# ChumpChief/FluidFramework

Hardware: AMD Instinct MI355X
Metric: sequenced ops applied/sec (whole node) + achieved HBM GB/s, conflict-farm replay (higher is better)
Workload: dtype int32

## Files before the change

### fluidframework_amd/csrc/kernels.h

```cpp
#pragma once

#include <hip/hip_runtime.h>

#include "../../include/fmt.h"

namespace fmt_mt {
struct AdjustTables;
struct LocalTables;
}

namespace fmt_kernels {

size_t mapLwwLdsBytes(uint32_t keyBound);
bool mapLwwNeedsScratch(uint32_t keyBound);
size_t mapSparseLdsBytes();
hipError_t launchMapSparse(const fmt_map_op* ops, const uint64_t* offsets, uint32_t nDocs, uint32_t keyBound,
                           fmt_map_entry* out, uint32_t* counts, int* error, int numCUs, hipStream_t stream);
hipError_t launchMapSparsePack(const fmt_map_entry* in, const uint64_t* offsets, const uint32_t* counts,
                               const uint64_t* packedOff, uint32_t nDocs, fmt_map_entry* packed, hipStream_t stream);
size_t mapPendingScratchBytes(uint64_t nEvents);
hipError_t launchMapPending(const fmt_map_local_op* events, const uint64_t* evOffs, const fmt_map_entry* seqEntries,
                            const uint64_t* seqOffs, const uint32_t* seqCounts, uint32_t nDocs, void* scratch,
                            const uint64_t* outBase, fmt_map_entry* out, uint32_t* outCounts, int32_t* outStatus,
                            hipStream_t stream);
// ... 5 lines not shown
  const uint64_t* docOpOffsets;
  uint32_t nDocs;
  const uint16_t* text;
  const uint32_t* docInit;
  const uint32_t* propsOff;
  const uint32_t* propsKv;
  uint32_t nPropsOps;
  const uint64_t* catchupOffsets;
  const fmt_mt_snapshot_doc* snapshots;
  const fmt_mt_snapshot_seg* snapshotSegs;
  const uint64_t* rmOrderOffsets;
  const fmt_mt_snapshot_info* snapshotInfo;
  const fmt_mt_stamp* snapshotStamps;
  uint64_t nSnapshotInfo;
  const fmt_mt_relpos* relpos;
  uint32_t nRelpos;
  uint32_t markerKey;
  const fmt_mt::AdjustTables* adj;
  const fmt_mt::LocalTables* loc = nullptr;
};

struct MtDeviceOut {
  fmt_mt_doc_result* headers;
  fmt_mt_leaf* leaves;
  uint16_t* chars;
  fmt_mt_propset* props;
  fmt_mt_catchup_range* catchup;
  fmt_mt_remove_order* rmOrder;
  uint32_t* ckpt;
  const fmt_mt_leaf* smallLeaves;
  const uint16_t* smallChars;
  uint16_t* legacyProps;
  uint32_t* hugeCkpt = nullptr;
};
size_t mergeTreeCheckpointBytes();

struct SumView {
  const fmt_mt_leaf* leaves;
  const uint16_t* chars;
  const fmt_mt_propset* props;
  const uint16_t* legacyProps;
  const uint32_t* cls;
  const uint64_t* rmHi;
};
struct SumRun {
  uint32_t len;
  uint16_t props;
  uint16_t flags;
};
struct SumDocOut {
  unsigned long long run_off, text_off;
  uint32_t n_runs, n_units, status, pad;
};
hipError_t launchSummaryRuns(const fmt_mt_doc_result* hdrs, const SumView* views, uint32_t nDocs, SumRun* runs,
                             uint16_t* text, unsigned long long* cursors, SumDocOut* docOut, int numCUs,
                             hipStream_t stream);
struct GatherSpan {
  const uint32_t* src;
  uint64_t dstWord;
  uint32_t words, pad;
};
hipError_t launchGatherSpans(const GatherSpan* spans, uint32_t n, uint32_t* dst, int numCUs, hipStream_t stream);
hipError_t launchStateDigest(const fmt_mt_doc_result* hdrs, const SumView* views, uint32_t nDocs, uint64_t* out,
                             int numCUs, hipStream_t stream);

struct MtCaps {
  uint32_t leaves, chars, props;
};
MtCaps mergeTreeCaps(bool large);

hipError_t launchMergeTree(const MtDeviceBatch& batch, const MtDeviceOut& out, const uint32_t* docList,
                           uint32_t count, uint32_t* esc, uint32_t* esc2, uint32_t* esc3, uint32_t* esc4, int numCUs,
                           hipStream_t stream, bool obliterate, bool removeOrder, uint32_t* sched, bool adjust);

hipError_t launchMergeTreeLarge(const MtDeviceBatch& batch, const MtDeviceOut& out, const uint32_t* docList,
                                uint32_t count, int numCUs, hipStream_t stream, bool obliterate, bool removeOrder,
                                uint32_t* next, bool adjust, bool local = false);

hipError_t launchMergeTreeLocal(const MtDeviceBatch& batch, const MtDeviceOut& out, const uint32_t* docList,
                                uint32_t count, uint32_t* esc, uint32_t* esc2, int numCUs, hipStream_t stream,
                                uint32_t* sched, bool adjust = false);

int mergeTreeProfile(uint64_t* out, int n, bool reset);

}

namespace fmt_huge {
struct HugeState;
struct HugeInputs;
}

namespace fmt_kernels {

struct HugeOut {
  fmt_mt_doc_result* header;
  fmt_mt_leaf* leaves;
  uint64_t capLeaves;
  uint16_t* chars;
  uint64_t capChars;
  fmt_mt_propset* props;
  uint16_t* legacy;
  const uint32_t* cls;
  unsigned long long* prof;
  uint64_t* leavesHi;
};
size_t hugeLdsBytes();
// ... 5 lines not shown
```

### fluidframework_amd/csrc/mergetree.hip

```cpp
#define FMT_MT_COLLECT_DEFINE 1
#include "mergetree_kernel.h"

namespace fmt_kernels {

constexpr int kMtWaves = 4;

int mergeTreeProfileCompact(uint64_t* out, int n, bool reset);
int mergeTreeProfileMicro(uint64_t* out, int n, bool reset);
int mergeTreeProfileLarge(uint64_t* out, int n, bool reset);

int mergeTreeProfile(uint64_t* out, int n, bool reset) {
  for (int c = 0; c < n; c++) out[c] = 0;
  if (addTuProfile(out, n, reset) < 0 || mergeTreeProfileCompact(out, n, reset) < 0 ||
      mergeTreeProfileMicro(out, n, reset) < 0 || mergeTreeProfileLarge(out, n, reset) < 0)
    return -1;
  return fmt_mt::kPfCount;
}

MtCaps mergeTreeCaps(bool large) {
  if (large)
    return MtCaps{static_cast<uint32_t>(Slab<fmt_mt::LargeTier>::kLeaves), static_cast<uint32_t>(Slab<fmt_mt::LargeTier>::kChars),
                  static_cast<uint32_t>(Slab<fmt_mt::LargeTier>::kProps)};
  return MtCaps{static_cast<uint32_t>(Slab<fmt_mt::SmallTier>::kLeaves), static_cast<uint32_t>(Slab<fmt_mt::SmallTier>::kChars),
                static_cast<uint32_t>(Slab<fmt_mt::SmallTier>::kProps)};
}

size_t mergeTreeCheckpointBytes() { return sizeof(uint32_t) * fmt_mt::Doc<false, fmt_mt::CompactTier>::kCkptWords; }

hipError_t launchMergeTreeCompact(const MtDeviceBatch& batch, const MtDeviceOut& out, const uint32_t* docList,
                                  uint32_t count, uint32_t* esc, int numCUs, hipStream_t stream, uint32_t* next,
                                  bool obliterate, const uint32_t* countDev);
hipError_t launchMergeTreeMicro(const MtDeviceBatch& batch, const MtDeviceOut& out, const uint32_t* docList,
                                uint32_t count, uint32_t* esc, int numCUs, hipStream_t stream, uint32_t* next);

constexpr int kOrderBuckets = 64;
__global__ __launch_bounds__(1024) void orderByRemainingKernel(const uint32_t* __restrict__ in, uint32_t* __restrict__ out,
                                                               const fmt_mt_doc_result* __restrict__ headers,
                                                               const uint64_t* __restrict__ offs,
                                                               const uint32_t* __restrict__ ckpt, uint32_t ckptWords) {
  __shared__ uint32_t cnt[kOrderBuckets], base[kOrderBuckets], maxRem;
  const uint32_t n = in[0];
  if (threadIdx.x < kOrderBuckets) cnt[threadIdx.x] = 0;
  if (threadIdx.x == 0) maxRem = 0;
  __syncthreads();
  auto remaining = [&](uint32_t d) -> uint32_t {
    uint64_t first = offs[d];
    if (headers[d].status == fmt_mt::kCkptEscalate) {
      const uint32_t* h = ckpt + static_cast<size_t>(d) * ckptWords;
      first = h[0] | (static_cast<uint64_t>(h[1]) << 32);
    }
    const uint64_t r = offs[d + 1] - first;
    return r > 0xffffffffull ? 0xffffffffu : static_cast<uint32_t>(r);
  };
  for (uint32_t i = threadIdx.x; i < n; i += blockDim.x) atomicMax(&maxRem, remaining(in[1 + i]));
  __syncthreads();
  const uint64_t span = static_cast<uint64_t>(maxRem) + 1;
  auto bucket = [&](uint32_t r) -> uint32_t {
    return kOrderBuckets - 1 - static_cast<uint32_t>(static_cast<uint64_t>(r) * kOrderBuckets / span);
  };
  for (uint32_t i = threadIdx.x; i < n; i += blockDim.x) atomicAdd(&cnt[bucket(remaining(in[1 + i]))], 1u);
  __syncthreads();
  if (threadIdx.x == 0) {
    uint32_t s = 0;
    for (int b = 0; b < kOrderBuckets; b++) {
      base[b] = s;
      s += cnt[b];
    }
    out[0] = n;
  }
  __syncthreads();
  for (uint32_t i = threadIdx.x; i < n; i += blockDim.x) {
    const uint32_t d = in[1 + i];
    out[1 + atomicAdd(&base[bucket(remaining(d))], 1u)] = d;
  }
}

hipError_t launchMergeTree(const MtDeviceBatch& batch, const MtDeviceOut& out, const uint32_t* docList,
                           uint32_t count, uint32_t* esc, uint32_t* esc2, uint32_t* esc3, uint32_t* esc4, int numCUs,
                           hipStream_t stream, bool obliterate, bool removeOrder, uint32_t* sched, bool adjust) {
  using S = fmt_mt::SmallTier;
  uint32_t* n1 = sched ? sched + 1 : nullptr;
  if (adjust) {
    if (removeOrder)
      return launchTier<true, S, true, kMtWaves, 1, true>(batch, out, docList, count, esc, numCUs, stream, nullptr, n1);
    return launchTier<true, S, false, kMtWaves, 1, true>(batch, out, docList, count, esc, numCUs, stream, nullptr, n1);
  }
  if (obliterate && removeOrder)
    return launchTier<true, S, true, kMtWaves, 2>(batch, out, docList, count, esc, numCUs, stream, nullptr, n1);
  if (obliterate && (esc == nullptr || esc2 == nullptr))
    return launchTier<true, S, false, kMtWaves, 2>(batch, out, docList, count, esc, numCUs, stream, nullptr, n1);
  if (removeOrder)
    return launchTier<false, S, true, kMtWaves, 2>(batch, out, docList, count, esc, numCUs, stream, nullptr, n1);
  if (esc == nullptr || esc2 == nullptr)
    return launchTier<false, S, false, kMtWaves, 2>(batch, out, docList, count, esc, numCUs, stream, nullptr, n1);
  constexpr uint32_t kCkptWords = static_cast<uint32_t>(fmt_mt::Doc<false, fmt_mt::CompactTier>::kCkptWords);
  const bool order = esc3 != nullptr && out.ckpt != nullptr;
  hipError_t e;
  if (!obliterate && esc4 != nullptr) {
    e = launchMergeTreeMicro(batch, out, docList, count, esc2, numCUs, stream, sched ? sched + 3 : nullptr);
    if (e != hipSuccess) return e;
    uint32_t* list = esc2;
    if (order) {
      hipLaunchKernelGGL(orderByRemainingKernel, dim3(1), dim3(1024), 0, stream, esc2, esc3, out.headers,
                         batch.docOpOffsets, out.ckpt, kCkptWords);
      list = esc3;
    }
    e = launchMergeTreeCompact(batch, out, list + 1, count, esc4, numCUs, stream, sched, false, list);
    if (e != hipSuccess) return e;
    if (order) {
      hipLaunchKernelGGL(orderByRemainingKernel, dim3(1), dim3(1024), 0, stream, esc4, esc2, out.headers,
                         batch.docOpOffsets, out.ckpt, kCkptWords);
      list = esc2;
    } else {
      list = esc4;
    }
    return launchTier<false, S, false, kMtWaves, 2>(batch, out, list + 1, count, esc, numCUs, stream, list, n1);
  }
  e = launchMergeTreeCompact(batch, out, docList, count, esc2, numCUs, stream, sched, obliterate, nullptr);
  if (e != hipSuccess) return e;
  if (order) {
    hipLaunchKernelGGL(orderByRemainingKernel, dim3(1), dim3(1024), 0, stream, esc2, esc3, out.headers,
                       batch.docOpOffsets, out.ckpt, kCkptWords);
    esc2 = esc3;
  }
  if (obliterate)
    return launchTier<true, S, false, kMtWaves, 2>(batch, out, esc2 + 1, count, esc, numCUs, stream, esc2, n1);
  return launchTier<false, S, false, kMtWaves, 2>(batch, out, esc2 + 1, count, esc, numCUs, stream, esc2, n1);
}

}
```

### fluidframework_amd/csrc/mergetree_kernel.h

```cpp
#pragma once
#include <hip/hip_runtime.h>

#include "kernels.h"
#include "mt_engine.h"

namespace fmt_kernels {

static __device__ unsigned long long g_mtProfile[fmt_mt::kPfCount];

static inline int addTuProfile(uint64_t* out, int n, bool reset) {
  unsigned long long h[fmt_mt::kPfCount];
  if (hipMemcpyFromSymbol(h, HIP_SYMBOL(g_mtProfile), sizeof h) != hipSuccess) return -1;
  for (int c = 0; c < n && c < fmt_mt::kPfCount; c++) out[c] += h[c];
  if (reset) {
    unsigned long long z[fmt_mt::kPfCount] = {};
    if (hipMemcpyToSymbol(HIP_SYMBOL(g_mtProfile), z, sizeof z) != hipSuccess) return -1;
  }
  return fmt_mt::kPfCount;
}

template <class C>
struct Slab {
  static constexpr size_t kLeaves = C::kHbmChars ? 64 * C::kRows : 64 * fmt_mt::SmallTier::kRows;
  static constexpr size_t kChars = C::kHbmChars ? C::kCapChars : fmt_mt::SmallTier::kCapChars;
// ... 54 lines not shown
      in.snapSeq = sd.seq;
      in.loaded = 1;
    } else {
      in.snapSegs = nullptr;
      in.snapInfo = nullptr;
      in.snapStamps = nullptr;
      in.nHeader = in.nBody = 0;
      in.snapMinSeq = in.snapSeq = 0;
      in.loaded = 0;
    }
    fmt_mt::DocOutputs o;
    o.header = out.headers + d;
    o.leaves = out.leaves + slot * Slab<C>::kLeaves;
    o.chars = out.chars + slot * Slab<C>::kChars;
    o.props = out.props + slot * Slab<C>::kProps;
    if (batch.catchupOffsets) {
      const uint64_t c0 = batch.catchupOffsets[d], c1 = batch.catchupOffsets[d + 1];
      o.catchup = out.catchup + c0;
      o.catchupCap = static_cast<uint32_t>(c1 - c0);
    } else {
      o.catchup = nullptr;
      o.catchupCap = 0;
    }
    if (Rm && batch.rmOrderOffsets) {
      const uint64_t r0 = batch.rmOrderOffsets[d], r1 = batch.rmOrderOffsets[d + 1];
      o.rmOrder = out.rmOrder + r0;
      o.rmOrderCap = static_cast<uint32_t>(r1 - r0);
    } else {
      o.rmOrder = nullptr;
      o.rmOrderCap = 0;
    }
    if (Doc::kSavesCkpt || Doc::kResumesCkpt || (Ob && Doc::kResumesBig)) {
      o.ckpt = out.ckpt ? out.ckpt + static_cast<size_t>(d) * Doc::kCkptWords : nullptr;
      o.ckptResume = Doc::kResumesCkpt && (!Doc::kSavesCkpt || countDev != nullptr) && o.ckpt != nullptr &&
                     __builtin_amdgcn_readfirstlane(out.headers[d].status) == fmt_mt::kCkptEscalate;
    } else {
      o.ckpt = nullptr;
      o.ckptResume = false;
    }
    o.bigCkpt = nullptr;
    o.bigCkptChars = nullptr;
    o.legacyProps = out.legacyProps ? out.legacyProps + slot * Slab<C>::kLeaves : nullptr;
    o.hugeCkpt = Doc::kSavesHuge && out.hugeCkpt != nullptr ? out.hugeCkpt + slot * static_cast<size_t>(fmt_ckpt::kWords) : nullptr;
    if constexpr (Doc::kSavesBig) {
      if (out.ckpt != nullptr) {
        o.bigCkpt = reinterpret_cast<uint32_t*>(o.leaves);
        o.bigCkptChars = o.chars;
      }
    }
    if constexpr (Doc::kResumesBig) {
      if (out.smallLeaves != nullptr) {
        o.bigCkpt = const_cast<uint32_t*>(reinterpret_cast<const uint32_t*>(out.smallLeaves + d * Slab<fmt_mt::SmallTier>::kLeaves));
        o.bigCkptChars = const_cast<uint16_t*>(out.smallChars + d * Slab<fmt_mt::SmallTier>::kChars);
        o.ckptResume = __builtin_amdgcn_readfirstlane(out.headers[d].status) == fmt_mt::kCkptEscalate;
      }
    }
    Doc doc;
    doc.s = scratch;
    doc.run(in, o);
#if FMT_PROFILE && FMT_GPU
    if ((threadIdx.x & 63) == 0)
      for (int c = 0; c < fmt_mt::kPfCount; c++) atomicAdd(&g_mtProfile[c], static_cast<unsigned long long>(doc.prof[c]));
#endif
  }
}

__global__ __launch_bounds__(256) void collectOverflowKernel(fmt_mt_doc_result* __restrict__ headers,
                                                             const uint32_t* __restrict__ docList, uint32_t nDocs,
                                                             const uint32_t* countDev, uint32_t* esc);

#ifdef FMT_MT_COLLECT_DEFINE
__global__ __launch_bounds__(256) void collectOverflowKernel(fmt_mt_doc_result* __restrict__ headers,
                                                             const uint32_t* __restrict__ docList, uint32_t nDocs,
                                                             const uint32_t* countDev, uint32_t* esc) {
  if (countDev != nullptr) nDocs = *countDev;
  for (uint32_t i = blockIdx.x * blockDim.x + threadIdx.x; i < nDocs; i += gridDim.x * blockDim.x) {
    const uint32_t d = docList ? docList[i] : i;
    const int st = headers[d].status;
    if (st == fmt_mt::kCapacityFinal) headers[d].status = FMT_E_CAPACITY;
    if (st == FMT_E_CAPACITY || st == fmt_mt::kCkptEscalate) {
      const uint32_t k = atomicAdd(esc, 1u);
      esc[1 + k] = d;
    }
  }
}
#endif

template <bool Ob, class C, bool Rm, int Waves, int WavesPerEU, bool Adj = false, bool Loc = false>
static hipError_t launchTier(const MtDeviceBatch& batch, const MtDeviceOut& out, const uint32_t* docList,
                             uint32_t count, uint32_t* esc, int numCUs, hipStream_t stream,
                             const uint32_t* countDev = nullptr, uint32_t* next = nullptr) {
  const size_t lds = scratchBytes<C, Ob>() * Waves;
  int blocksPerCU = 0;
  const hipError_t e =
      hipOccupancyMaxActiveBlocksPerMultiprocessor(&blocksPerCU, mergeTreeKernel<Ob, C, Rm, Waves, WavesPerEU, Adj, Loc>, 64 * Waves, lds);
  if (e != hipSuccess) return e;
  const uint32_t wanted = (count + Waves - 1) / Waves;
  const uint32_t cap = static_cast<uint32_t>(numCUs * (blocksPerCU > 0 ? blocksPerCU : 1));
  const uint32_t grid = wanted < cap ? (wanted > 0 ? wanted : 1) : cap;
  hipLaunchKernelGGL((mergeTreeKernel<Ob, C, Rm, Waves, WavesPerEU, Adj, Loc>), dim3(grid), dim3(64 * Waves), lds, stream, batch, out,
                     docList, count, countDev, next);
  if (esc != nullptr) {
    const uint32_t g = (count + 255) / 256;
    hipLaunchKernelGGL(collectOverflowKernel, dim3(g < 1024 ? (g > 0 ? g : 1) : 1024), dim3(256), 0, stream, out.headers,
                       docList, count, countDev, esc);
  }
  return hipGetLastError();
}

}
```

### fluidframework_amd/csrc/mt_engine.h

```cpp
#pragma once

#include "../../include/fmt.h"
#include "wave.h"
#include "adjust.h"
#include "huge_ckpt.h"

#include <cstddef>
#include <type_traits>

#if FMT_GPU
#define FMT_LDS __attribute__((address_space(3)))
#else
#define FMT_LDS
#endif

namespace fmt_mt {

constexpr int kMaxNodes = 8;
constexpr int kGranularity = 256;
constexpr int kObCap = 64;
constexpr int kKeysMax = FMT_MT_PROPS_KEYS_MAX;
constexpr int kKeyChunks = kKeysMax / 64;
static_assert(kKeysMax % 64 == 0, "prop-set slots come in whole waves");
constexpr int32_t kNotRemoved = 0x7fffffff;
constexpr int kCapacityFinal = -33;
constexpr int kCkptEscalate = -34;

struct SmallTier {
  static constexpr int kRows = 8;
  static constexpr int kCapChars = 6144;
  static constexpr int kMaxBlocks = 128;
  static constexpr int kHeapCap = 255;
  static constexpr int kPropCap = 32;
  static constexpr int kLenBits = 16, kBlkBits = 8;
  static constexpr bool kHbmChars = false;
  static constexpr bool kUnroll = true;
  static constexpr int kWords = 5;
  static constexpr int kMaxClient = 31;
  static constexpr bool kPropsWord = false;
  using BId = uint8_t;
  using VR = V8;
};

struct CompactTier : SmallTier {
  static constexpr int kRows = 4;
  static constexpr int kCapChars = 2048;
  using VR = V4;
};

struct MicroTier : SmallTier {
  static constexpr int kRows = 2;
  static constexpr int kCapChars = 1024;
  using VR = V2;
};

struct LargeTier {
  static constexpr int kRows = 32;
  static constexpr int kCapChars = 131071;
  static constexpr int kMaxBlocks = 1023;
// ... 98 lines not shown
  uint32_t nPropsOps;
  const fmt_mt_snapshot_seg* snapSegs;
  uint32_t nHeader, nBody;
  int32_t snapMinSeq, snapSeq;
  uint32_t loaded;
  const fmt_mt_snapshot_info* snapInfo;
  const fmt_mt_stamp* snapStamps;
  const fmt_mt_snapshot_info* infoAll;
  const fmt_mt_stamp* stampsAll;
  uint64_t nInfoAll;
  const fmt_mt_relpos* relpos;
  uint32_t nRelpos;
  uint32_t markerKey;
  const AdjustTables* adj;
  uint32_t doc;
  const LocalTables* loc = nullptr;
};

struct DocOutputs {
  fmt_mt_doc_result* header;
  fmt_mt_leaf* leaves;
  uint16_t* chars;
  fmt_mt_propset* props;
  fmt_mt_catchup_range* catchup;
  uint32_t catchupCap;
  fmt_mt_remove_order* rmOrder;
  uint32_t rmOrderCap;
  uint32_t* ckpt;
  bool ckptResume;
  uint32_t* bigCkpt;
  uint16_t* bigCkptChars;
  uint16_t* legacyProps;
  uint32_t* hugeCkpt = nullptr;
};

#ifndef FMT_PROFILE
#define FMT_PROFILE 0
#endif
#ifndef FMT_SCALAR_OPS
#define FMT_SCALAR_OPS 0
#endif
enum ProfCat {
  kPfOpLoad, kPfScan, kPfSplit, kPfInsert, kPfRange, kPfLru, kPfZamboniOp, kPfWindow, kPfOutput,
  kPfInsChars, kPfInsShift, kPfZFind, kPfZChars, kPfZSerial, kPfZDelete, kPfZPack, kPfCount
};

template <bool Ob, class C = SmallTier, bool Rm = false, bool Adj = false, bool Loc = false>
class Doc {
 public:
  using VR = typename C::VR;
  using BId = typename C::BId;
  static constexpr int kRows = C::kRows;
  static constexpr int kRowUnroll = C::kUnroll ? C::kRows : 1;
  static constexpr int kCapLeaves = 64 * kRows;
  static constexpr int kCapChars = C::kCapChars;
  static constexpr int kMaxBlocks = C::kMaxBlocks;
  static constexpr int kHeapCap = C::kHeapCap;
  static constexpr int kPropCap = C::kPropCap;
  static constexpr uint32_t kLenMask = (1u << C::kLenBits) - 1u;
  static constexpr uint32_t kNoBlk = (1u << C::kBlkBits) - 1u;
  static constexpr bool kPW = C::kPropsWord;
  static constexpr int kCapFinal = C::kHbmChars ? FMT_E_CAPACITY : kCapacityFinal;
  static constexpr uint32_t kPropsUndef = kPW ? 0xFFFFu : (1u << (32 - C::kLenBits - C::kBlkBits)) - 1u;
  static_assert(kMaxBlocks <= static_cast<int>(kNoBlk) && kPropCap <= static_cast<int>(kPropsUndef), "W0 field widths");
  static_assert(kRows <= 32, "row bitmasks are 32-bit");
  FMT_DEV static uint32_t fLen(uint32_t w0) { return w0 & kLenMask; }
// ... 22 lines not shown
  Lane<VR> W[kWords];
  FMT_LDS Scratch<C>* s;
  uint16_t* gch = nullptr;
  int n = 0;
  int nChars = 0;
  int root = 0;
  int nFree = 0;
  int heapN = 0;
  int nProps = 0;
  int curSeq = 0;
  int minSeq = 0;
  int status = FMT_OK;
  int failSeq = 0;
  uint32_t nextId = 1;
  uint32_t opIdx = 0;
  int obSeqN = 0;
  int obStartN = 0;
  uint64_t obUsed = 0;
  uint32_t cuN = 0;
  DocInputs in;
  fmt_mt_catchup_range* cuOut = nullptr;
  uint32_t cuCap = 0;
  uint32_t rmN = 0;
  fmt_mt_remove_order* rmOut = nullptr;
  uint32_t rmCap = 0;
  int rmPendN = 0;
  uint32_t rmPendFrom0 = 0, rmPendTo0 = 0, rmPendFrom1 = 0, rmPendTo1 = 0;
  bool rmHitsSet = false;
  Lane<uint32_t> rmHits;

  static constexpr bool kRegTier = !C::kHbmChars && !Rm && !Loc;
  static constexpr bool kSavesCkpt = kRegTier && C::kRows < SmallTier::kRows;
  static constexpr bool kResumesCkpt = kRegTier && (C::kRows == SmallTier::kRows || (C::kRows > MicroTier::kRows && !Ob));
  static constexpr int kCkptRows = CompactTier::kRows;
  static constexpr int kCkptHead = 16;
  static constexpr int kCkptCharWords = CompactTier::kCapChars / 2;
  static constexpr int kCkptRestWords =
      static_cast<int>((offsetof(Scratch<CompactTier>, tmp) - offsetof(Scratch<CompactTier>, blk) + 3) / 4);
  static_assert(offsetof(Scratch<CompactTier>, tmp) - offsetof(Scratch<CompactTier>, blk) ==
                    offsetof(Scratch<SmallTier>, tmp) - offsetof(Scratch<SmallTier>, blk),
                "checkpointed scratch fields");
  static constexpr int kCkptObWords =
      static_cast<int>((offsetof(Scratch<CompactTier>, obStart) + kObCap - offsetof(Scratch<CompactTier>, ob) + 3) / 4);
  static_assert(offsetof(Scratch<CompactTier>, obStart) - offsetof(Scratch<CompactTier>, ob) ==
                    offsetof(Scratch<SmallTier>, obStart) - offsetof(Scratch<SmallTier>, ob),
                "checkpointed obliterate fields");
  static constexpr int kCkptWords = kCkptHead + 5 * kCkptRows * 64 + kCkptCharWords + kCkptRestWords + kCkptObWords;
  uint32_t* ckpt = nullptr;
  uint64_t ckptNext = 0;

  static constexpr bool kSavesBig = !C::kHbmChars && C::kRows == SmallTier::kRows && !Rm && !Loc;
  static constexpr bool kResumesBig = C::kHbmChars && !Rm && !Loc;
  static constexpr int kCkptObOff = kCkptWords - kCkptObWords;
  static constexpr int kBigRows = SmallTier::kRows;
  static constexpr int kBigRestWords =
      static_cast<int>((offsetof(Scratch<SmallTier>, tmp) - offsetof(Scratch<SmallTier>, blk) + 3) / 4);
  static_assert(kCkptHead + 5 * kBigRows * 64 + kBigRestWords <= 64 * SmallTier::kRows * 8,
                "the small tier's checkpoint fits its leaves slab");
  uint32_t* bigCkpt = nullptr;
  uint16_t* bigCkptChars = nullptr;

  static constexpr bool kSavesHuge = C::kHbmChars && !Loc;
  uint32_t* hugeCkpt = nullptr;
  bool savingHuge = false;
  FMT_DEV void saveHuge(uint64_t next) {
    namespace K = fmt_ckpt;
// ... 3298 lines not shown
      if (bad != FMT_OK) fail(bad);
      else if (loader) loadBodySegment(op, text);
      else if (Loc && (op.flags & FMT_MT_F_ACK)) ackOp(op);
      else if ((op.flags & (FMT_MT_F_REL1 | FMT_MT_F_REL2)) == 0 || resolveRelative(op)) applyOp(op, text);
      if constexpr (Rm) {
        if (rmPendN > 0 || rmHitsSet)
          rmFlush(op.client, op.seq, op.type == FMT_MT_REMOVE ? FMT_MT_RM_SET : FMT_MT_RM_SLICE);
      }
      const bool lastMember = !loader && (i + 1 == in.end || (recWord(rec0, 7) & (FMT_MT_F_GROUP_CONT | FMT_MT_F_LOADSEG)) !=
                                                                 FMT_MT_F_GROUP_CONT);
      for (int z = 0; z < 2 && status == FMT_OK; z++) {
        if (z == 1) {
          if (!lastMember) break;
          if (curSeq > op.seq || op.min_seq > op.seq || minSeq > op.min_seq) {
            fail(FMT_E_DATA);
            break;
          }
          curSeq = op.seq;
          int eff = op.min_seq;
          if constexpr (Loc) {
            if (gHead < gTail && static_cast<int32_t>(gWord(gHead, 4)) < eff) eff = static_cast<int32_t>(gWord(gHead, 4));
          }
          if (eff <= minSeq) break;
          minSeq = eff;
          if constexpr (Ob) obSetMinSeq();
        }
        zamboni();
        stamp(z == 0 ? kPfZamboniOp : kPfWindow);
      }
      if (status != FMT_OK) {
        failSeq = op.seq;
        break;
      }
    }
  }

  FMT_DEV void writeOutputs(const DocOutputs& out) {
    if constexpr (Loc) {
      FOR_LANES(l) {
        if (l < 2) storeGlobal(in.loc->regenCount + 2 * in.doc + l, l == 0 ? regenN : regenTextN);
      }
    }
    if constexpr (Adj) {
      if (out.legacyProps != nullptr && status == FMT_OK && !savingHuge) {
        pmLegacyProps(out.legacyProps);
        if (status != FMT_OK) {
          if constexpr (C::kHbmChars) {
            status = FMT_OK;
            FOR_LANES(l) {
              for (int t = l; t < n; t += 64) out.legacyProps[t] = kLegacyUnavailable;
            }
            waveSync();
          } else {
            status = FMT_E_CAPACITY;
          }
        }
      }
    }
    const int nr = rows();
    Lane<VR> cst;
    charStarts(cst, nr);
    Lane<VR> startFlag, ord;
    FOR_ROWS(r, 0, nr) {
      const Lane<uint32_t> cur = row(W[0], r);
      const Lane<uint32_t> up = shflUp1(cur);
      const uint32_t carry = r > 0 ? readlane(row(W[0], r > 0 ? r - 1 : 0), 63) : 0u;
// ... 91 lines not shown

    rmOut = out.rmOrder;
    rmCap = out.rmOrder ? out.rmOrderCap : 0u;
    rmN = 0;
    if constexpr (C::kHbmChars) gch = out.chars;
    ckpt = out.ckpt;
    init();
    uint64_t first = in.begin;
    bigCkpt = out.bigCkpt;
    bigCkptChars = out.bigCkptChars;
    if (kResumesCkpt && ckpt != nullptr && out.ckptResume) {
      first = restoreCkpt();
    } else if (kResumesBig && bigCkpt != nullptr && out.ckptResume) {
      first = restoreBig();
    } else {
      if (in.adj != nullptr) {
        FOR_LANES(l) {
          if (l == 0) storeGlobal(in.adj->numCount + in.doc, 0u);
        }
      }
      pmN = 0;
      if constexpr (Loc) {
        locSeq = 0;
        gHead = gTail = 0;
        recN = 0;
        recFrozen = false;
        regenN = regenTextN = 0;
        normSet = false;
      }
      if (in.loaded) loadSnapshot();
      else loadInitial();
    }
    hugeCkpt = out.hugeCkpt;
    if (status == FMT_OK) replay(first);
    if constexpr (kSavesHuge) {
      if (status == kCkptEscalate) {
        status = FMT_OK;
        savingHuge = true;
        writeOutputs(out);
        saveHuge(ckptNext);
        FOR_LANES(l) {
          if (l == 0) out.header->status = fmt_ckpt::kStatusHuge;
        }
        return;
      }
    }
    if ((kSavesCkpt || kSavesBig) && status == kCkptEscalate) {
      if constexpr (!Ob && kSavesCkpt) saveCkpt(ckptNext);
      else if constexpr (!Ob && kSavesBig) saveBig(ckptNext);
      FOR_LANES(l) {
        if (l == 0) out.header->status = status;
      }
      return;
    }
    writeOutputs(out);
    stamp(kPfOutput);
  }
};

}
```

### fluidframework_amd/csrc/runtime.cpp

```cpp
#include <hip/hip_runtime.h>

#include <algorithm>
#include <chrono>
#include <cstdio>
#include <thread>
#include <cstring>
#include <exception>
#include <string>
#include <vector>

#include "../../include/fmt.h"
#include "huge_engine.h"
#include "jsnum.h"
#include "mt_engine.h"
#include "kernels.h"

namespace {

template <class T>
struct DevBuf {
  T* p = nullptr;
  size_t cap = 0;
  hipError_t reserve(size_t n) {
    if (n <= cap && p != nullptr) return hipSuccess;
// ... 78 lines not shown
  DevBuf<fmt_map_slot> mapOut;
  DevBuf<uint32_t> mapScratch;
  DevBuf<int> errWord;
  uint64_t mapNOps = 0;
  uint32_t mapDocs = 0, mapKeyBound = 0;
  bool mapLoaded = false;
  DevBuf<fmt_map_entry> mapEntries, mapPacked;
  DevBuf<uint32_t> mapCounts;
  DevBuf<uint64_t> mapPackedOff;
  bool mapSparse = false;
  bool mapSparseRan = false;
  std::vector<uint64_t> mapOffsHost;
  DevBuf<fmt_map_local_op> mapEv;
  DevBuf<uint64_t> mapEvOffs, mapPendBase;
  DevBuf<uint8_t> mapPendScratch;
  DevBuf<fmt_map_entry> mapPendOut;
  DevBuf<uint32_t> mapPendCounts;
  DevBuf<int32_t> mapPendStatus;
  bool mapPendRan = false;

  DevBuf<fmt_mt_op> mtOps;
  DevBuf<uint64_t> mtOffs;
  DevBuf<uint16_t> mtText;
  DevBuf<uint32_t> mtInit, mtPropsOff, mtPropsKv;
  DevBuf<fmt_mt_doc_result> mtHdr;
  DevBuf<fmt_mt_leaf> mtLeaves;
  DevBuf<uint16_t> mtChars;
  DevBuf<fmt_mt_propset> mtProps;
  DevBuf<uint32_t> mtEsc;
  DevBuf<uint32_t> mtEsc2;
  DevBuf<uint32_t> mtEsc3;
  DevBuf<uint32_t> mtEsc4;
  DevBuf<uint32_t> mtCkpt;
  DevBuf<uint32_t> mtHugeCk;
  bool mtCkptOk = false;
  DevBuf<uint32_t> mtSched;
  DevBuf<fmt_mt_leaf> mtBigLeaves;
  DevBuf<uint16_t> mtBigChars;
  DevBuf<fmt_mt_propset> mtBigProps;
  std::vector<int32_t> mtBigSlot;
  DevBuf<fmt_mt_snapshot_doc> mtSnap;
  DevBuf<fmt_mt_snapshot_seg> mtSnapSegs;
  DevBuf<fmt_mt_relpos> mtRelpos;
  DevBuf<fmt_mt_snapshot_info> mtSnapInfo;
  DevBuf<fmt_mt_stamp> mtSnapStamps;
  bool mtHasSnapInfo = false;
  uint64_t mtNSnapSegs = 0;
  uint32_t mtNRelpos = 0, mtMarkerKey = FMT_MT_NO_MARKER;
  bool mtHasSnap = false;
  bool mtObliterate = false;
  DevBuf<uint64_t> mtCuOffs;
  DevBuf<fmt_mt_catchup_range> mtCatchup;
  std::vector<uint64_t> mtCuOffsHost;
  bool mtHasCatchup = false;
  DevBuf<uint64_t> mtRmOffs;
  DevBuf<fmt_mt_remove_order> mtRmOrder;
  std::vector<uint64_t> mtRmOffsHost;
  bool mtHasRmOrder = false;
  struct HugeDocBufs {
    std::vector<void*> allocs;
    fmt_huge::HugeState state{};
    fmt_huge::HugeInputs in{};
    fmt_kernels::HugeOut out{};
    std::vector<uint32_t> shape;
  };
  std::vector<HugeDocBufs> huge;
// ... 209 lines not shown
  if (c->stream) (void)hipStreamSynchronize(c->stream);
  c->mapOps.release();
  c->mapOffs.release();
  c->mapOut.release();
  c->mapScratch.release();
  c->mapEntries.release();
  c->mapPacked.release();
  c->mapEv.release();
  c->mapEvOffs.release();
  c->mapPendBase.release();
  c->mapPendScratch.release();
  c->mapPendOut.release();
  c->mapPendCounts.release();
  c->mapPendStatus.release();
  c->mapCounts.release();
  c->mapPackedOff.release();
  c->errWord.release();
  c->mtOps.release();
  c->mtOffs.release();
  c->mtText.release();
  c->mtInit.release();
  c->mtPropsOff.release();
  c->mtPropsKv.release();
  c->mtHdr.release();
  c->mtLeaves.release();
  c->mtChars.release();
  c->mtProps.release();
  c->mtEsc.release();
  c->mtEsc2.release();
  c->mtEsc3.release();
  c->mtEsc4.release();
  c->mtSched.release();
  c->mtCkpt.release();
  c->mtHugeCk.release();
  c->mtBigLeaves.release();
  c->mtBigChars.release();
  c->mtBigProps.release();
  c->mtSnap.release();
  c->mtSnapSegs.release();
  c->mtRelpos.release();
  c->mtSnapInfo.release();
  c->mtSnapStamps.release();
  c->mtCuOffs.release();
  c->mtCatchup.release();
  c->mtRmOffs.release();
  c->mtRmOrder.release();
  for (auto& h : c->huge)
    for (void* p : h.allocs) (void)hipFree(p);
  c->huge.clear();
  c->mtSmallList.release();
  c->hugeStates.release();
  c->hugeInputs.release();
  c->hugeOuts.release();
  c->stage.release();
  c->mtPm.release();
  c->mtPmOffs.release();
  c->mtLegacy.release();
  c->mtBigLegacy.release();
  for (auto* q : {&c->mtLocGroups, &c->mtLocRecs, &c->mtLocPm, &c->mtLocScratch, &c->mtLocRegenCount}) q->release();
  c->mtLocOffs.release();
  c->mtLocRegen.release();
  c->mtLocRegenText.release();
  c->mtLocTab.release();
  c->spans.release();
  c->packed.release();
  c->digests.release();
// ... 794 lines not shown
    for (uint64_t k = 0; k < b->n_snapshot_segs && !c->mtHiClients; k++) c->mtHiClients = b->snapshot_info[k].ins_client > 63;
  }
  c->mtNRelpos = b->relpos ? b->n_relpos : 0u;
  c->mtMarkerKey = b->marker_id_key;
  if (c->mtNRelpos) {
    FMT_HIP(c, c->mtRelpos.reserve(c->mtNRelpos));
    FMT_HIP(c, cp(c->mtRelpos.p, b->relpos, c->mtNRelpos * sizeof(fmt_mt_relpos)));
  }
  if (c->mtHasCatchup) FMT_HIP(c, cp(c->mtCuOffs.p, c->mtCuOffsHost.data(), (n + 1ull) * sizeof(uint64_t)));
  if (c->mtHasRmOrder) FMT_HIP(c, cp(c->mtRmOffs.p, c->mtRmOffsHost.data(), (n + 1ull) * sizeof(uint64_t)));
  if (b->props_off) {
    FMT_HIP(c, cp(c->mtPropsOff.p, b->props_off, (b->n_props_ops + 1ull) * sizeof(uint32_t)));
    FMT_HIP(c, cp(c->mtPropsKv.p, b->props_kv, nKv * sizeof(uint32_t)));
  } else {
    FMT_HIP(c, hipMemsetAsync(c->mtPropsOff.p, 0, sizeof(uint32_t), c->stream));
  }
  FMT_HIP(c, hipStreamSynchronize(c->stream));
  c->mtNOps = b->n_ops;
  c->mtDocs = n;
  c->mtTextLen = b->text_len;
  c->mtNPropsOps = b->n_props_ops;
  c->mtOffsHost.assign(b->doc_op_offsets, b->doc_op_offsets + n + 1);
  if (b->snapshots) c->mtSnapHost.assign(b->snapshots, b->snapshots + n);
  else c->mtSnapHost.clear();
  c->mtNProps = b->n_props_ops;
  c->mtHasInit = b->doc_init != nullptr;
  c->mtObliterate = obliterates;
  c->mtCkptOk = false;
  if (!c->mtHasRmOrder) {
    c->mtCkptOk = c->mtCkpt.reserve(static_cast<size_t>(n) * (fmt_kernels::mergeTreeCheckpointBytes() / sizeof(uint32_t))) ==
                  hipSuccess;
    if (!c->mtCkptOk) (void)hipGetLastError();
  }
  c->mtInsertChars = insertChars;
  c->mtInitChars = initChars;
  for (auto& h : c->huge)
    for (void* p : h.allocs) (void)hipFree(p);
  c->huge.clear();
  c->mtHugeSlot.assign(n, -1);
  c->mtHugeOk.assign(n, 1);
  c->mtLoadSegs.assign(n, 0);
  c->mtSegProps.assign(n, 0);
  c->mtDocChars.assign(n, 0);
  c->mtStartSeg.assign(n, fmt_mt_snapshot_seg{0, 0, FMT_MT_NO_PROPS});
  parallelChunks(n, [&](uint64_t d0, uint64_t d1, unsigned) {
  for (uint64_t d = d0; d < d1; d++) {
    uint8_t ok = 1;
    uint64_t chars = 0;
    uint32_t loadSegs = 0;
    for (uint64_t i = b->doc_op_offsets[d]; i < b->doc_op_offsets[d + 1]; i++) {
      const fmt_mt_op& op = b->ops[i];
      if (op.type == FMT_MT_INSERT) chars += fmt_mt_op_len(&op);
      if (op.flags & FMT_MT_F_LOADSEG) loadSegs++;
    }
    c->mtLoadSegs[d] = loadSegs;
    if (b->snapshots && b->snapshots[d].loaded) {
      const fmt_mt_snapshot_doc& sd = b->snapshots[d];
      for (uint64_t k = sd.first_seg; k < sd.first_seg + sd.n_header + sd.n_body; k++)
        if (b->snapshot_segs[k].props != FMT_MT_NO_PROPS) {
          c->mtSegProps[d] = 1;
          break;
        }
      for (uint64_t k = sd.first_seg; k < sd.first_seg + sd.n_header + sd.n_body; k++)
        chars += b->snapshot_segs[k].len & ~FMT_MT_SEG_MARKER;
    } else if (b->doc_init && b->doc_init[2 * d + 1] > 0) {
      c->mtStartSeg[d] = fmt_mt_snapshot_seg{b->doc_init[2 * d], b->doc_init[2 * d + 1], FMT_MT_NO_PROPS};
// ... 72 lines not shown
  FMT_HIP(c, hipStreamSynchronize(c->stream));
  c->mtLoaded = true;
  return FMT_OK;
}

int fmt_mt_run(fmt_ctx* c) {
  if (c == nullptr || !c->mtLoaded) return setErr(c, FMT_E_USAGE, "fmt_mt_run before fmt_mt_load");
  FMT_HIP(c, hipSetDevice(c->device));
  FMT_HIP(c, hipStreamSynchronize(c->stream));
  for (size_t h = c->mtHugeLoaded; h < c->huge.size(); h++)
    for (void* q : c->huge[h].allocs) (void)hipFree(q);
  for (uint32_t d = 0; d < c->mtDocs; d++)
    if (c->mtHugeSlot[d] >= static_cast<int32_t>(c->mtHugeLoaded)) c->mtHugeSlot[d] = -1;
  c->huge.resize(c->mtHugeLoaded);
  fmt_kernels::MtDeviceBatch db{c->mtOps.p, c->mtOffs.p, c->mtDocs, c->mtText.p,
                                c->mtHasInit ? c->mtInit.p : nullptr, c->mtPropsOff.p, c->mtPropsKv.p, c->mtNProps,
                                c->mtHasCatchup ? c->mtCuOffs.p : nullptr,
                                c->mtHasSnap ? c->mtSnap.p : nullptr, c->mtHasSnap ? c->mtSnapSegs.p : nullptr,
                                c->mtHasRmOrder ? c->mtRmOffs.p : nullptr,
                                c->mtHasSnapInfo ? c->mtSnapInfo.p : nullptr, c->mtHasSnapInfo ? c->mtSnapStamps.p : nullptr,
                                c->mtHasSnapInfo ? c->mtNSnapSegs : 0u,
                                c->mtNRelpos ? c->mtRelpos.p : nullptr,
                                c->mtNRelpos, c->mtMarkerKey,
                                c->mtHasAdjust ? c->mtAdjTab.p : nullptr,
                                c->mtLocal ? c->mtLocTab.p : nullptr};
  fmt_kernels::MtDeviceOut dout{c->mtHdr.p, c->mtLeaves.p, c->mtChars.p, c->mtProps.p,
                                c->mtHasCatchup ? c->mtCatchup.p : nullptr, c->mtHasRmOrder ? c->mtRmOrder.p : nullptr,
                                !c->mtHasRmOrder && !c->mtHasAdjust && c->mtCkptOk ? c->mtCkpt.p : nullptr, nullptr, nullptr,
                                c->mtHasAdjust ? c->mtLegacy.p : nullptr};
  FMT_HIP(c, hipMemsetAsync(c->mtEsc.p, 0, sizeof(uint32_t), c->stream));
  FMT_HIP(c, hipMemsetAsync(c->mtEsc2.p, 0, sizeof(uint32_t), c->stream));
  FMT_HIP(c, hipMemsetAsync(c->mtEsc4.p, 0, sizeof(uint32_t), c->stream));
  FMT_HIP(c, hipMemsetAsync(c->mtSched.p, 0, 4 * sizeof(uint32_t), c->stream));
  FMT_HIP(c, hipEventRecord(c->ev0, c->stream));
  const bool hasHuge = c->mtHugeLoaded > 0, list = c->mtUseList;
  if (c->mtLocal) {
    if (!list || c->mtNSmall > 0)
      FMT_HIP(c, fmt_kernels::launchMergeTreeLocal(db, dout, list ? c->mtSmallList.p : nullptr, list ? c->mtNSmall : c->mtDocs,
                                                   c->mtEsc.p, c->mtEsc2.p, c->numCUs, c->stream, c->mtSched.p,
                                                   c->mtHasAdjust));
  } else if (!list || c->mtNSmall > 0)
    FMT_HIP(c, fmt_kernels::launchMergeTree(db, dout, list ? c->mtSmallList.p : nullptr, list ? c->mtNSmall : c->mtDocs,
                                            c->mtEsc.p, c->mtEsc2.p, c->mtEsc3.p, c->mtEsc4.p, c->numCUs, c->stream,
                                            c->mtObliterate,
                                            c->mtHasRmOrder, c->mtSched.p, c->mtHasAdjust));
  if (hasHuge)
    FMT_HIP(c, fmt_kernels::launchHugeDocs(c->hugeStates.p, c->hugeInputs.p, c->hugeOuts.p, c->mtHugeLoaded, c->mtHasAdjust, c->mtHasRmOrder, c->stream));
  FMT_HIP(c, hipEventRecord(c->ev1, c->stream));
  c->timed2 = false;
  uint32_t nEsc = 0;
  c->mtGrown = 0;
  FMT_HIP(c, hipMemcpyAsync(&nEsc, c->mtEsc.p, sizeof nEsc, hipMemcpyDeviceToHost, c->stream));
  FMT_HIP(c, hipStreamSynchronize(c->stream));
  c->mtBigSlot.assign(c->mtDocs, -1);
  if (nEsc > 0) {
    const fmt_kernels::MtCaps big = fmt_kernels::mergeTreeCaps(true);
    FMT_HIP(c, c->mtBigLeaves.reserve(static_cast<size_t>(nEsc) * big.leaves));
    FMT_HIP(c, c->mtBigChars.reserve(static_cast<size_t>(nEsc) * big.chars));
    FMT_HIP(c, c->mtBigProps.reserve(static_cast<size_t>(nEsc) * big.props));
    if (c->mtHasAdjust) FMT_HIP(c, c->mtBigLegacy.reserve(static_cast<size_t>(nEsc) * big.leaves));
    const bool hugeCk = !c->mtLocal &&
                        c->mtHugeCk.reserve(static_cast<size_t>(nEsc) * fmt_ckpt::kWords) == hipSuccess;
    if (!hugeCk) (void)hipGetLastError();
    fmt_kernels::MtDeviceOut bout{c->mtHdr.p, c->mtBigLeaves.p, c->mtBigChars.p, c->mtBigProps.p,
                                  c->mtHasCatchup ? c->mtCatchup.p : nullptr, c->mtHasRmOrder ? c->mtRmOrder.p : nullptr,
                                  c->mtObliterate && !c->mtHasRmOrder && !c->mtHasAdjust && c->mtCkptOk ? c->mtCkpt.p : nullptr,
                                  !c->mtHasRmOrder ? c->mtLeaves.p : nullptr, !c->mtHasRmOrder ? c->mtChars.p : nullptr,
                                  c->mtHasAdjust ? c->mtBigLegacy.p : nullptr, hugeCk ? c->mtHugeCk.p : nullptr};
    FMT_HIP(c, hipEventRecord(c->ev2, c->stream));
    FMT_HIP(c, fmt_kernels::launchMergeTreeLarge(db, bout, c->mtEsc.p + 1, nEsc, c->numCUs, c->stream, c->mtObliterate,
                                                 c->mtHasRmOrder, c->mtSched.p + 2, c->mtHasAdjust, c->mtLocal));
    FMT_HIP(c, hipEventRecord(c->ev3, c->stream));
    c->timed2 = true;
    std::vector<uint32_t> list(nEsc);
    FMT_HIP(c, hipMemcpyAsync(list.data(), c->mtEsc.p + 1, nEsc * sizeof(uint32_t), hipMemcpyDeviceToHost, c->stream));
    FMT_HIP(c, hipStreamSynchronize(c->stream));
    for (uint32_t i = 0; i < nEsc; i++) c->mtBigSlot[list[i]] = static_cast<int32_t>(i);
    std::vector<fmt_mt_doc_result> hb(nEsc);
// ... 609 lines not shown
```

Before: 519.0 million.

## Step documents down from small tier back to compact tier when they shrink

Adds a descend path. A document replaying in the small register tier can checkpoint and hand itself back to the cheaper compact tier once its leaf, char and prop counts fall well below compact capacity and enough ops remain. The launch now loops over multiple compact→small rounds with per-round doc lists held in a new device buffer, and the collect kernel routes descending docs into the next round. This is meant to avoid running shrunken docs on the heavier, lower-occupancy tier for the rest of their ops, at the cost of extra kernel launches, a checkpoint save/restore per descent, and an extra memset.

```diff
diff --git a/fluidframework_amd/csrc/kernels.h b/fluidframework_amd/csrc/kernels.h
--- a/fluidframework_amd/csrc/kernels.h
+++ b/fluidframework_amd/csrc/kernels.h
@@ -61,6 +61,7 @@
   const uint16_t* smallChars;
   uint16_t* legacyProps;
   uint32_t* hugeCkpt = nullptr;
+  bool descend = false;
 };
 size_t mergeTreeCheckpointBytes();
 
@@ -100,7 +101,9 @@
 
 hipError_t launchMergeTree(const MtDeviceBatch& batch, const MtDeviceOut& out, const uint32_t* docList,
                            uint32_t count, uint32_t* esc, uint32_t* esc2, uint32_t* esc3, uint32_t* esc4, int numCUs,
-                           hipStream_t stream, bool obliterate, bool removeOrder, uint32_t* sched, bool adjust);
+                           hipStream_t stream, bool obliterate, bool removeOrder, uint32_t* sched, bool adjust,
+                           uint32_t* desc = nullptr);
+size_t mergeTreeDescendWords(uint32_t count);
 
 hipError_t launchMergeTreeLarge(const MtDeviceBatch& batch, const MtDeviceOut& out, const uint32_t* docList,
                                 uint32_t count, int numCUs, hipStream_t stream, bool obliterate, bool removeOrder,
diff --git a/fluidframework_amd/csrc/mergetree.hip b/fluidframework_amd/csrc/mergetree.hip
--- a/fluidframework_amd/csrc/mergetree.hip
+++ b/fluidframework_amd/csrc/mergetree.hip
@@ -33,6 +33,16 @@
 hipError_t launchMergeTreeMicro(const MtDeviceBatch& batch, const MtDeviceOut& out, const uint32_t* docList,
                                 uint32_t count, uint32_t* esc, int numCUs, hipStream_t stream, uint32_t* next);
 
+#ifndef FMT_DESCEND_ROUNDS
+#define FMT_DESCEND_ROUNDS 2
+#endif
+constexpr int kDescendRounds = FMT_DESCEND_ROUNDS;
+constexpr size_t kDescendHead = 64;
+
+size_t mergeTreeDescendWords(uint32_t count) {
+  return kDescendHead + static_cast<size_t>(2 * (kDescendRounds - 1)) * (static_cast<size_t>(count) + 1);
+}
+
 constexpr int kOrderBuckets = 64;
 __global__ __launch_bounds__(1024) void orderByRemainingKernel(const uint32_t* __restrict__ in, uint32_t* __restrict__ out,
                                                                const fmt_mt_doc_result* __restrict__ headers,
@@ -45,7 +55,7 @@
   __syncthreads();
   auto remaining = [&](uint32_t d) -> uint32_t {
     uint64_t first = offs[d];
-    if (headers[d].status == fmt_mt::kCkptEscalate) {
+    if (headers[d].status == fmt_mt::kCkptEscalate || headers[d].status == fmt_mt::kCkptDescend) {
       const uint32_t* h = ckpt + static_cast<size_t>(d) * ckptWords;
       first = h[0] | (static_cast<uint64_t>(h[1]) << 32);
     }
@@ -77,7 +87,8 @@
 
 hipError_t launchMergeTree(const MtDeviceBatch& batch, const MtDeviceOut& out, const uint32_t* docList,
                            uint32_t count, uint32_t* esc, uint32_t* esc2, uint32_t* esc3, uint32_t* esc4, int numCUs,
-                           hipStream_t stream, bool obliterate, bool removeOrder, uint32_t* sched, bool adjust) {
+                           hipStream_t stream, bool obliterate, bool removeOrder, uint32_t* sched, bool adjust,
+                           uint32_t* desc) {
   using S = fmt_mt::SmallTier;
   uint32_t* n1 = sched ? sched + 1 : nullptr;
   if (adjust) {
@@ -97,24 +108,33 @@
   const bool order = esc3 != nullptr && out.ckpt != nullptr;
   hipError_t e;
   if (!obliterate && esc4 != nullptr) {
+    const int rounds = order && desc != nullptr ? kDescendRounds : 1;
+    const size_t stride = static_cast<size_t>(count) + 1;
+    const auto roundList = [&](int r, int k) { return desc + kDescendHead + (static_cast<size_t>(2 * (r - 1) + k)) * stride; };
+    const auto ordered = [&](uint32_t* list) {
+      if (!order) return list;
+      hipLaunchKernelGGL(orderByRemainingKernel, dim3(1), dim3(1024), 0, stream, list, esc3, out.headers,
+                         batch.docOpOffsets, out.ckpt, kCkptWords);
+      return esc3;
+    };
     e = launchMergeTreeMicro(batch, out, docList, count, esc2, numCUs, stream, sched ? sched + 3 : nullptr);
     if (e != hipSuccess) return e;
-    uint32_t* list = esc2;
-    if (order) {
-      hipLaunchKernelGGL(orderByRemainingKernel, dim3(1), dim3(1024), 0, stream, esc2, esc3, out.headers,
-                         batch.docOpOffsets, out.ckpt, kCkptWords);
-      list = esc3;
+    for (int r = 0; r < rounds; r++) {
+      MtDeviceOut o = out;
+      o.descend = r + 1 < rounds;
+      uint32_t* toCompact = r == 0 ? esc2 : roundList(r, 0);
+      uint32_t* toSmall = r == 0 ? esc4 : roundList(r, 1);
+      uint32_t* down = o.descend ? roundList(r + 1, 0) : nullptr;
+      uint32_t* deal = sched && r > 0 ? desc + 2 * (r - 1) : nullptr;
+      const uint32_t* list = ordered(toCompact);
+      e = launchMergeTreeCompact(batch, o, list + 1, count, toSmall, numCUs, stream, r == 0 ? sched : deal, false, list);
+      if (e != hipSuccess) return e;
+      list = ordered(toSmall);
+      e = launchTier<false, S, false, kMtWaves, 2>(batch, o, list + 1, count, esc, numCUs, stream, list,
+                                                   r == 0 ? n1 : (deal ? deal + 1 : nullptr), down);
+      if (e != hipSuccess) return e;
     }
-    e = launchMergeTreeCompact(batch, out, list + 1, count, esc4, numCUs, stream, sched, false, list);
-    if (e != hipSuccess) return e;
-    if (order) {
-      hipLaunchKernelGGL(orderByRemainingKernel, dim3(1), dim3(1024), 0, stream, esc4, esc2, out.headers,
-                         batch.docOpOffsets, out.ckpt, kCkptWords);
-      list = esc2;
-    } else {
-      list = esc4;
-    }
-    return launchTier<false, S, false, kMtWaves, 2>(batch, out, list + 1, count, esc, numCUs, stream, list, n1);
+    return hipSuccess;
   }
   e = launchMergeTreeCompact(batch, out, docList, count, esc2, numCUs, stream, sched, obliterate, nullptr);
   if (e != hipSuccess) return e;
diff --git a/fluidframework_amd/csrc/mergetree_kernel.h b/fluidframework_amd/csrc/mergetree_kernel.h
--- a/fluidframework_amd/csrc/mergetree_kernel.h
+++ b/fluidframework_amd/csrc/mergetree_kernel.h
@@ -110,8 +110,10 @@
     }
     if (Doc::kSavesCkpt || Doc::kResumesCkpt || (Ob && Doc::kResumesBig)) {
       o.ckpt = out.ckpt ? out.ckpt + static_cast<size_t>(d) * Doc::kCkptWords : nullptr;
+      const int st = __builtin_amdgcn_readfirstlane(out.headers[d].status);
       o.ckptResume = Doc::kResumesCkpt && (!Doc::kSavesCkpt || countDev != nullptr) && o.ckpt != nullptr &&
-                     __builtin_amdgcn_readfirstlane(out.headers[d].status) == fmt_mt::kCkptEscalate;
+                     (st == fmt_mt::kCkptEscalate || (!Ob && st == fmt_mt::kCkptDescend));
+      if constexpr (Doc::kDescends) o.descend = out.descend;
     } else {
       o.ckpt = nullptr;
       o.ckptResume = false;
@@ -145,12 +147,12 @@
 
 __global__ __launch_bounds__(256) void collectOverflowKernel(fmt_mt_doc_result* __restrict__ headers,
                                                              const uint32_t* __restrict__ docList, uint32_t nDocs,
-                                                             const uint32_t* countDev, uint32_t* esc);
+                                                             const uint32_t* countDev, uint32_t* esc, uint32_t* down);
 
 #ifdef FMT_MT_COLLECT_DEFINE
 __global__ __launch_bounds__(256) void collectOverflowKernel(fmt_mt_doc_result* __restrict__ headers,
                                                              const uint32_t* __restrict__ docList, uint32_t nDocs,
-                                                             const uint32_t* countDev, uint32_t* esc) {
+                                                             const uint32_t* countDev, uint32_t* esc, uint32_t* down) {
   if (countDev != nullptr) nDocs = *countDev;
   for (uint32_t i = blockIdx.x * blockDim.x + threadIdx.x; i < nDocs; i += gridDim.x * blockDim.x) {
     const uint32_t d = docList ? docList[i] : i;
@@ -159,6 +161,9 @@
     if (st == FMT_E_CAPACITY || st == fmt_mt::kCkptEscalate) {
       const uint32_t k = atomicAdd(esc, 1u);
       esc[1 + k] = d;
+    } else if (down != nullptr && st == fmt_mt::kCkptDescend) {
+      const uint32_t k = atomicAdd(down, 1u);
+      down[1 + k] = d;
     }
   }
 }
@@ -167,7 +172,7 @@
 template <bool Ob, class C, bool Rm, int Waves, int WavesPerEU, bool Adj = false, bool Loc = false>
 static hipError_t launchTier(const MtDeviceBatch& batch, const MtDeviceOut& out, const uint32_t* docList,
                              uint32_t count, uint32_t* esc, int numCUs, hipStream_t stream,
-                             const uint32_t* countDev = nullptr, uint32_t* next = nullptr) {
+                             const uint32_t* countDev = nullptr, uint32_t* next = nullptr, uint32_t* down = nullptr) {
   const size_t lds = scratchBytes<C, Ob>() * Waves;
   int blocksPerCU = 0;
   const hipError_t e =
@@ -181,7 +186,7 @@
   if (esc != nullptr) {
     const uint32_t g = (count + 255) / 256;
     hipLaunchKernelGGL(collectOverflowKernel, dim3(g < 1024 ? (g > 0 ? g : 1) : 1024), dim3(256), 0, stream, out.headers,
-                       docList, count, countDev, esc);
+                       docList, count, countDev, esc, down);
   }
   return hipGetLastError();
 }
diff --git a/fluidframework_amd/csrc/mt_engine.h b/fluidframework_amd/csrc/mt_engine.h
--- a/fluidframework_amd/csrc/mt_engine.h
+++ b/fluidframework_amd/csrc/mt_engine.h
@@ -25,6 +25,9 @@
 constexpr int32_t kNotRemoved = 0x7fffffff;
 constexpr int kCapacityFinal = -33;
 constexpr int kCkptEscalate = -34;
+constexpr int kCkptDescend = -36;
+constexpr int kDescendLeaves4 = 128, kDescendChars4 = 1024;
+constexpr int kDescendMinOps = 128;
 
 struct SmallTier {
   static constexpr int kRows = 8;
@@ -189,6 +192,7 @@
   uint16_t* bigCkptChars;
   uint16_t* legacyProps;
   uint32_t* hugeCkpt = nullptr;
+  bool descend = false;
 };
 
 #ifndef FMT_PROFILE
@@ -277,6 +281,14 @@
   static constexpr bool kRegTier = !C::kHbmChars && !Rm && !Loc;
   static constexpr bool kSavesCkpt = kRegTier && C::kRows < SmallTier::kRows;
   static constexpr bool kResumesCkpt = kRegTier && (C::kRows == SmallTier::kRows || (C::kRows > MicroTier::kRows && !Ob));
+  static constexpr bool kDescends = kRegTier && !Ob && !Adj && C::kRows == SmallTier::kRows;
+  static constexpr int kDescendLeaves = kDescendLeaves4;
+  static constexpr int kDescendChars = kDescendChars4;
+  static_assert(SmallTier::kMaxBlocks == CompactTier::kMaxBlocks && SmallTier::kPropCap == CompactTier::kPropCap &&
+                    SmallTier::kMaxClient == CompactTier::kMaxClient && SmallTier::kHeapCap == CompactTier::kHeapCap &&
+                    2 * kDescendLeaves4 <= 64 * CompactTier::kRows && 2 * kDescendChars4 <= CompactTier::kCapChars,
+                "a document that steps down fits the compact tier with half of it to spare");
+  bool descend = false;
   static constexpr int kCkptRows = CompactTier::kRows;
   static constexpr int kCkptHead = 16;
   static constexpr int kCkptCharWords = CompactTier::kCapChars / 2;
@@ -3641,6 +3653,14 @@
         failSeq = op.seq;
         break;
       }
+      if constexpr (kDescends) {
+        if (descend && lastMember && n <= kDescendLeaves && nChars <= kDescendChars && nFree >= 16 &&
+            nProps <= kPropCap - 4 && i + 1 + kDescendMinOps <= in.end) {
+          ckptNext = i + 1;
+          status = kCkptDescend;
+          return;
+        }
+      }
     }
   }
 
@@ -3798,6 +3818,7 @@
       else loadInitial();
     }
     hugeCkpt = out.hugeCkpt;
+    if constexpr (kDescends) descend = out.descend && ckpt != nullptr;
     if (status == FMT_OK) replay(first);
     if constexpr (kSavesHuge) {
       if (status == kCkptEscalate) {
@@ -3811,6 +3832,15 @@
         return;
       }
     }
+    if constexpr (kDescends) {
+      if (status == kCkptDescend) {
+        saveCkpt(ckptNext);
+        FOR_LANES(l) {
+          if (l == 0) out.header->status = status;
+        }
+        return;
+      }
+    }
     if ((kSavesCkpt || kSavesBig) && status == kCkptEscalate) {
       if constexpr (!Ob && kSavesCkpt) saveCkpt(ckptNext);
       else if constexpr (!Ob && kSavesBig) saveBig(ckptNext);
diff --git a/fluidframework_amd/csrc/runtime.cpp b/fluidframework_amd/csrc/runtime.cpp
--- a/fluidframework_amd/csrc/runtime.cpp
+++ b/fluidframework_amd/csrc/runtime.cpp
@@ -134,6 +134,8 @@
   DevBuf<uint32_t> mtEsc3;
   DevBuf<uint32_t> mtEsc4;
   DevBuf<uint32_t> mtCkpt;
+  DevBuf<uint32_t> mtDesc;
+  size_t mtDescWords = 0;
   DevBuf<uint32_t> mtHugeCk;
   bool mtCkptOk = false;
   DevBuf<uint32_t> mtSched;
@@ -409,6 +411,7 @@
   c->mtEsc4.release();
   c->mtSched.release();
   c->mtCkpt.release();
+  c->mtDesc.release();
   c->mtHugeCk.release();
   c->mtBigLeaves.release();
   c->mtBigChars.release();
@@ -1269,6 +1272,12 @@
                   hipSuccess;
     if (!c->mtCkptOk) (void)hipGetLastError();
   }
+  c->mtDescWords = 0;
+  if (c->mtCkptOk && !obliterates && !c->mtHasAdjust && !c->mtLocal) {
+    const size_t words = fmt_kernels::mergeTreeDescendWords(n);
+    if (c->mtDesc.reserve(words) == hipSuccess) c->mtDescWords = words;
+    else (void)hipGetLastError();
+  }
   c->mtInsertChars = insertChars;
   c->mtInitChars = initChars;
   for (auto& h : c->huge)
@@ -1407,6 +1416,7 @@
   FMT_HIP(c, hipMemsetAsync(c->mtEsc2.p, 0, sizeof(uint32_t), c->stream));
   FMT_HIP(c, hipMemsetAsync(c->mtEsc4.p, 0, sizeof(uint32_t), c->stream));
   FMT_HIP(c, hipMemsetAsync(c->mtSched.p, 0, 4 * sizeof(uint32_t), c->stream));
+  if (c->mtDescWords > 0) FMT_HIP(c, hipMemsetAsync(c->mtDesc.p, 0, c->mtDescWords * sizeof(uint32_t), c->stream));
   FMT_HIP(c, hipEventRecord(c->ev0, c->stream));
   const bool hasHuge = c->mtHugeLoaded > 0, list = c->mtUseList;
   if (c->mtLocal) {
@@ -1418,7 +1428,8 @@
     FMT_HIP(c, fmt_kernels::launchMergeTree(db, dout, list ? c->mtSmallList.p : nullptr, list ? c->mtNSmall : c->mtDocs,
                                             c->mtEsc.p, c->mtEsc2.p, c->mtEsc3.p, c->mtEsc4.p, c->numCUs, c->stream,
                                             c->mtObliterate,
-                                            c->mtHasRmOrder, c->mtSched.p, c->mtHasAdjust));
+                                            c->mtHasRmOrder, c->mtSched.p, c->mtHasAdjust,
+                                            c->mtDescWords > 0 ? c->mtDesc.p : nullptr));
   if (hasHuge)
     FMT_HIP(c, fmt_kernels::launchHugeDocs(c->hugeStates.p, c->hugeInputs.p, c->hugeOuts.p, c->mtHugeLoaded, c->mtHasAdjust, c->mtHasRmOrder, c->stream));
   FMT_HIP(c, hipEventRecord(c->ev1, c->stream));
```

New measurement: 534.8 million, median of 6. 1.03x the previous value.
